# Tesla-Albert/Hybrid-Grid-for-Hexagonal-and-Rectangular-Image-Processing

Measured on AMD Instinct MI355X. Metric: Mpix/s rect→hex→rect+hexconv, 4K batch=128, 1/2/4/8 GPU; %HBM roofline, higher is better.
Workload: dtype bf16

## Files before the change

hybrid-grid-for-hexagonal-and-rectangular-image-processing_amd/csrc/fused4.hip:

```cpp
#include <climits>
#include <cmath>
#include <cstdlib>

#include "fused_kernel.h"

namespace hg {

#ifndef F4_RB_
#define F4_RB_ 30
#endif
#ifndef F4_PD
#define F4_PD 2
#endif
#ifndef F4_WPS
#define F4_WPS 29
#endif
#ifndef F4_ORDER
#define F4_ORDER 0
#endif
#ifndef F4_WPE
#define F4_WPE 3
#endif
#ifndef F4_REV
#define F4_REV 1
#endif
constexpr int F4_GW = 4, F4_THREADS = 256;
constexpr int F4_HL = 8, F4_OWN = 240;
constexpr int F4_RB = F4_RB_;
static_assert(F4_RB % 6 == 0 && F4_RB > 0, "bands are whole 6-step blocks");

typedef unsigned f4_u2 __attribute__((ext_vector_type(2)));

__device__ __forceinline__ void f4_unpack(f4_u2 r, fu_f2& a, fu_f2& b, unsigned hi16) {
    a = fu_f2{__builtin_bit_cast(float, r.x << 16), __builtin_bit_cast(float, r.x & hi16)};
    b = fu_f2{__builtin_bit_cast(float, r.y << 16), __builtin_bit_cast(float, r.y & hi16)};
}

template <int OP>
__global__ __launch_bounds__(F4_THREADS) __attribute__((amdgpu_waves_per_eu(F4_WPE)))
void k_fused4(const __bf16* __restrict__ x, const float* __restrict__ kern,
              const float* __restrict__ bias, __bf16* __restrict__ y, FusedGeom F) {
    constexpr int C = 3, O = 3;
    constexpr int PD = F4_PD;
    static_assert(PD >= 1 && PD <= 4, "raw ring: rows k+2 .. k+1+PD in flight in 6 slots");
    constexpr int RB = F4_RB, NLUT = RB + 2;
    __shared__ float4 lut_all[F4_GW][NLUT];
    const int lane = threadIdx.x & 63;
    const int wslot = __builtin_amdgcn_readfirstlane(threadIdx.x >> 6);
    float4* const lut = lut_all[wslot];
    const int64_t blk = (int64_t)xcd_swizzle(blockIdx.x, gridDim.x);
    const int ngrp = (F.nwin + F4_GW - 1) / F4_GW;
    const int grp = (int)(F4_ORDER == 1 ? (blk / F.nband) % ngrp : blk % ngrp);
    const int band = (int)(F4_ORDER == 1 ? blk % F.nband : (blk / ngrp) % F.nband);
    const int64_t b = blk / ((int64_t)ngrp * F.nband);
    if (b >= F.B) return;
    const int win = grp * F4_GW + wslot;
    const int W0 = win * F4_OWN - F4_HL;
    const int ce = W0 + 4 * lane;
    const int s0 = band * RB;
    const int s1 = min(s0 + RB, F.h2);
    const bool up = F4_REV && (band & 1) && s1 - s0 == RB;

    for (int e = lane; e < NLUT; e += 64) {
        const int r = s0 - 1 + e;
        float4 t = {0.f, 0.f, 0.f, 0.f};
        if (r >= 0 && r < F.h1) {
            const double i_ = axis_at(F.rxs, r) + (double)(F.h - 1) * 0.5;
            const int in = (int)i_;
            const double f = i_ - (double)(float)in;
            const float w0 = (in >= 0 && in < F.h) ? (float)(1.0 - f) : 0.f;
            const float w1 = (in + 1 >= 0 && in + 1 < F.h) ? (float)f : 0.f;
            if (in == r - 1) { t.x = w0; t.y = w1; }
            else if (in == r) { t.y = w0; t.z = w1; }
        }
        lut[e] = t;
    }
    __builtin_amdgcn_s_waitcnt(0xc07f);
    __builtin_amdgcn_wave_barrier();
    int rc;
    {
        bool has_a = false, has_c = false;
        for (int e = lane; e < NLUT; e += 64) {
            const float4 t = lut[e];
            has_a |= t.x != 0.f;
            has_c |= t.z != 0.f;
        }
        const bool any_a = __builtin_amdgcn_ballot_w64(has_a) != 0;
        const bool any_c = __builtin_amdgcn_ballot_w64(has_c) != 0;
        rc = !any_c ? 1 : (!any_a ? 2 : 0);
    }

    float we[2][3], wo[2][3];
#pragma unroll
    for (int k = 0; k < 2; ++k)
#pragma unroll
        for (int s = 0; s < 2; ++s) {
            float* wr = s ? wo[k] : we[k];
            wr[0] = wr[1] = wr[2] = 0.f;
            const int q = ce + 2 * k + s;
            if (q >= 0 && q < F.w1) {
                const double j_ = axis_at(F.rys, q) + (double)(F.w - 1) * 0.5;
                const int jn = (int)j_;
                const double jf = j_ - (double)(float)jn;
#pragma unroll
                for (int kk = -1; kk <= 1; ++kk) {
                    const bool in_w = q + kk >= 0 && q + kk < F.w;
                    if (kk == jn - q && in_w) wr[kk + 1] += (float)(1.0 - jf);
                    if (kk == jn + 1 - q && in_w) wr[kk + 1] += (float)jf;
                }
            }
#pragma unroll
            for (int t = 0; t < 3; ++t) wr[t] *= 0.75f;
        }
    const bool any_l = __builtin_amdgcn_ballot_w64(we[0][0] != 0.f || wo[0][0] != 0.f ||
                                                   we[1][0] != 0.f || wo[1][0] != 0.f) != 0;
    const bool any_r = __builtin_amdgcn_ballot_w64(we[0][2] != 0.f || wo[0][2] != 0.f ||
                                                   we[1][2] != 0.f || wo[1][2] != 0.f) != 0;
    const int cd = !any_r ? 1 : (!any_l ? 2 : 0);

    const bool own = lane >= F4_HL / 4 && lane < (F4_HL + F4_OWN) / 4 && ce >= 0 && ce < F.w2 &&
                     win < F.nwin;

    const int64_t cstride = (int64_t)F.h * F.w, ostride = (int64_t)F.h2 * F.w2;
    const __amdgpu_buffer_rsrc_t xrs = __builtin_amdgcn_make_buffer_rsrc(
        (void*)(x + b * C * cstride), (short)0, (int)(C * cstride * 2), 0x00020000);
    const __amdgpu_buffer_rsrc_t yrs = __builtin_amdgcn_make_buffer_rsrc(
        (void*)(y + b * O * ostride), (short)0, (int)(O * ostride * 2), 0x00020000);
    const int lc = min(max(ce, 0), F.w - 4);
    const unsigned xoff = (unsigned)lc * 2u;
    const unsigned yoff = own ? (unsigned)ce * 2u : 0x80000000u;
    const unsigned xplane = (unsigned)(cstride * 2), yplane = (unsigned)(ostride * 2);
    const unsigned xrow = (unsigned)F.w * 2u, yrow = (unsigned)F.w2 * 2u;
    auto row_off = [&](int r) -> unsigned {
        return (unsigned)__builtin_amdgcn_readfirstlane((int)((unsigned)min(max(r, 0), F.h - 1) * xrow));
    };

    int vz = 0;
    asm volatile("" : "+v"(vz));
    constexpr int NW = O * C * 7, NWP = (NW + 1) / 2;
    constexpr int NWS = F4_WPS < NWP ? F4_WPS : NWP;
    float wk[NW];
#pragma unroll
    for (int i = 0; i < NW; ++i) wk[i] = kern[i + (i / 2 < NWS ? 0 : vz)];
    fu_f2 wkp[NWP];
#pragma unroll
    for (int i = 0; i < NWP; ++i) {
        wkp[i] = fu_f2{wk[2 * i], 2 * i + 1 < NW ? wk[2 * i + 1] : 0.f};
        if (i >= NWS) asm volatile("" : "+v"(wkp[i]));
    }
    float bv[O];
#pragma unroll
    for (int o = 0; o < O; ++o) bv[o] = bias ? bias[o + vz] * 0.75f : 0.f;
    fu_f2 bvp[2];
#pragma unroll
    for (int i = 0; i < 2; ++i) {
        bvp[i] = fu_f2{bv[2 * i], 2 * i + 1 < O ? bv[2 * i + 1] : 0.f};
        asm volatile("" : "+v"(bvp[i]));
    }
    float c13 = 1.f / 3.f;
    asm volatile("" : "+v"(c13));
    const float wn_f = (ce + 4 < F.w2) ? c13 : 0.f;
    const float wp_f = (ce - 1 >= 0) ? c13 : 0.f;
    unsigned hi16 = 0xffff0000u;
    asm volatile("" : "+v"(hi16));

    auto run = [&](auto CDc, auto RCc, auto UPc) {
        constexpr int CD = decltype(CDc)::value;
        constexpr int RC = decltype(RCc)::value;
        constexpr bool UP = decltype(UPc)::value;
        auto row = [&](int k) { return UP ? s1 - 1 - k : s0 + k; };
        auto lut_e = [&](int j) { return UP ? RB - j : j + 1; };
        f4_u2 raw[6][C];
        fu_f2 XA[3][C], XB[3][C];
        fu_f2 ZA[3][O], ZB[3][O];

        auto issue = [&](auto SLc, int r, bool live = true) {
            constexpr int SL = decltype(SLc)::value;
            const unsigned so = row_off(r);
            const unsigned vo = live ? xoff : 0x80000000u;
#pragma unroll
            for (int c = 0; c < C; ++c) raw[SL][c] = __builtin_amdgcn_raw_buffer_load_b64(xrs, vo, so + c * xplane, 0);
        };
        auto convert = [&](auto RSc, auto XSc) {
            constexpr int RS = decltype(RSc)::value, XS = decltype(XSc)::value;
#pragma unroll
            for (int c = 0; c < C; ++c) f4_unpack(raw[RS][c], XA[XS][c], XB[XS][c], hi16);
        };

        auto urow = [&](auto PHc, float4 L, auto CENc, auto BELc) {
            constexpr int PH = decltype(PHc)::value;
            constexpr bool CEN = decltype(CENc)::value, BEL = decltype(BELc)::value;
            constexpr int S0 = fu_mod(PH, 3), S1 = fu_mod(PH + 1, 3), S2 = fu_mod(PH + 2, 3);
            constexpr int XM = UP ? S2 : S0, XQ = UP ? S0 : S2;
            constexpr int PB = UP ? fu_mod(PH + 1, 2) : fu_mod(PH, 2), PC = 1 - PB;
            constexpr int TN = UP ? 5 : 0, TD = UP ? 0 : 5;
            const fu_f2 Lxy = {L.x, L.y}, Lzw = {L.z, L.w};
            fu_sfor<0, C>([&](auto Cc) {
                constexpr int c = decltype(Cc)::value;
                float ue[2], uo[2];
                auto vblend = [&](const fu_f2 (&X)[3][C]) {
                    if constexpr (RC == 1) return fu_pfma<1, false>(Lxy, X[S1][c], fu_pmul<0>(Lxy, X[XM][c]));
                    else if constexpr (RC == 2) return fu_pfma<0, false>(Lzw, X[XQ][c], fu_pmul<1>(Lxy, X[S1][c]));
                    else return fu_pfma<0, false>(Lzw, X[XQ][c], fu_pfma<1, false>(Lxy, X[S1][c], fu_pmul<0>(Lxy, X[XM][c])));
                };
                const fu_f2 VA = vblend(XA), VB = vblend(XB);
                if constexpr (CD == 1) {
                    ue[0] = fmaf(we[0][1], VA.x, we[0][0] * f_prev(VB.y));
                    uo[0] = fmaf(wo[0][1], VA.y, wo[0][0] * VA.x);
                    ue[1] = fmaf(we[1][1], VB.x, we[1][0] * VA.y);
                    uo[1] = fmaf(wo[1][1], VB.y, wo[1][0] * VB.x);
                } else if constexpr (CD == 2) {
                    ue[0] = fmaf(we[0][2], VA.y, we[0][1] * VA.x);
                    uo[0] = fmaf(wo[0][2], VB.x, wo[0][1] * VA.y);
                    ue[1] = fmaf(we[1][2], VB.y, we[1][1] * VB.x);
                    uo[1] = fmaf(wo[1][2], f_next(VA.x), wo[1][1] * VB.y);
                } else {
                    const float pl = f_prev(VB.y), nx = f_next(VA.x);
                    ue[0] = fmaf(we[0][2], VA.y, fmaf(we[0][1], VA.x, we[0][0] * pl));
                    uo[0] = fmaf(wo[0][2], VB.x, fmaf(wo[0][1], VA.y, wo[0][0] * VA.x));
                    ue[1] = fmaf(we[1][2], VB.y, fmaf(we[1][1], VB.x, we[1][0] * VA.y));
                    uo[1] = fmaf(wo[1][2], nx, fmaf(wo[1][1], VB.y, wo[1][0] * VB.x));
                }
                const float nue = f_next(ue[0]);
                const fu_f2 U0[2] = {fu_f2{ue[0], uo[0]}, fu_f2{ue[1], uo[1]}};
                const fu_f2 U1[2] = {fu_f2{uo[0], ue[1]}, fu_f2{uo[1], nue}};
                const fu_f2 Um[2] = {fu_f2{f_prev(uo[1]), ue[0]}, fu_f2{uo[0], ue[1]}};
                const fu_f2 U2[2] = {U0[1], fu_f2{nue, OP == 0 ? f_next(uo[0]) : 0.f}};
                fu_sfor<0, O>([&](auto OOc) {
                    constexpr int o = decltype(OOc)::value;
                    constexpr int j0 = (o * C + c) * 7;
                    auto tapk = [&](auto Tc, fu_f2& zA, fu_f2& zB, int par) {
                        constexpr int j = j0 + decltype(Tc)::value;
                        constexpr bool WS = (j >> 1) < NWS;
                        const int s = fu_tap_shift(decltype(Tc)::value, par, OP);
                        const fu_f2 aA = s == -1 ? Um[0] : (s == 0 ? U0[0] : (s == 1 ? U1[0] : U2[0]));
                        const fu_f2 aB = s == -1 ? Um[1] : (s == 0 ? U0[1] : (s == 1 ? U1[1] : U2[1]));
                        zA = fu_pfma<j & 1, WS>(wkp[j >> 1], aA, zA);
                        zB = fu_pfma<j & 1, WS>(wkp[j >> 1], aB, zB);
                    };
                    if constexpr (c == 0) {
                        constexpr int jb = j0 + TN;
                        constexpr bool WS = (jb >> 1) < NWS;
                        const int s = fu_tap_shift(TN, PB, OP);
                        const fu_f2 aA = s == -1 ? Um[0] : (s == 0 ? U0[0] : (s == 1 ? U1[0] : U2[0]));
                        const fu_f2 aB = s == -1 ? Um[1] : (s == 0 ? U0[1] : (s == 1 ? U1[1] : U2[1]));
                        ZA[S2][o] = fu_pfma_b<jb & 1, o & 1, WS>(wkp[jb >> 1], aA, bvp[o >> 1]);
                        ZB[S2][o] = fu_pfma_b<jb & 1, o & 1, WS>(wkp[jb >> 1], aB, bvp[o >> 1]);
                    } else {
                        tapk(IC<TN>{}, ZA[S2][o], ZB[S2][o], PB);
                    }
                    tapk(IC<TN + 1>{}, ZA[S2][o], ZB[S2][o], PB);
                    if constexpr (CEN) {
                        tapk(IC<2>{}, ZA[S1][o], ZB[S1][o], PC);
                        tapk(IC<3>{}, ZA[S1][o], ZB[S1][o], PC);
                        tapk(IC<4>{}, ZA[S1][o], ZB[S1][o], PC);
                    }
                    if constexpr (BEL) {
                        tapk(IC<TD>{}, ZA[S0][o], ZB[S0][o], PB);
                        tapk(IC<TD + 1>{}, ZA[S0][o], ZB[S0][o], PB);
                    }
                });
            });
        };

        auto out_row = [&](auto PHc, int k) {
            constexpr int PH = decltype(PHc)::value;
            constexpr int S0 = PH % 3;
            constexpr int PAR = UP ? (PH + 1) & 1 : PH & 1;
            const unsigned so = (unsigned)__builtin_amdgcn_readfirstlane((int)((unsigned)row(k) * yrow));
#pragma unroll
            for (int o = 0; o < O; ++o) {
                const fu_f2 zA = ZA[S0][o], zB = ZB[S0][o];
                float o0, o1, o2, o3;
                if constexpr (PAR == 0) {
                    o0 = fmaf(c13, zA.y, zA.x);
                    o1 = fmaf(c13, zB.x, zA.y);
                    o2 = fmaf(c13, zB.y, zB.x);
                    o3 = fmaf(wn_f, f_next(zA.x), zB.y);
                } else {
                    o0 = fmaf(wp_f, f_prev(zB.y), zA.x);
                    o1 = fmaf(c13, zA.x, zA.y);
                    o2 = fmaf(c13, zA.y, zB.x);
                    o3 = fmaf(c13, zB.x, zB.y);
                }
                typedef __bf16 t2v __attribute__((ext_vector_type(2)));
                const f4_u2 v = {__builtin_bit_cast(unsigned, t2v{(__bf16)o0, (__bf16)o1}),
                                 __builtin_bit_cast(unsigned, t2v{(__bf16)o2, (__bf16)o3})};
                __builtin_amdgcn_raw_buffer_store_b64(v, yrs, yoff, so + o * yplane, 0);
            }
        };

        {
            f4_u2 t0[C], t1[C], t2[C];
            const unsigned o0 = row_off(row(-2)), o1 = row_off(row(-1)), o2 = row_off(row(0));
#pragma unroll
            for (int c = 0; c < C; ++c) {
                t0[c] = __builtin_amdgcn_raw_buffer_load_b64(xrs, xoff, o0 + c * xplane, 0);
                t1[c] = __builtin_amdgcn_raw_buffer_load_b64(xrs, xoff, o1 + c * xplane, 0);
                t2[c] = __builtin_amdgcn_raw_buffer_load_b64(xrs, xoff, o2 + c * xplane, 0);
            }
            issue(IC<1>{}, row(1));
#pragma unroll
            for (int i = 0; i < PD; ++i) {
                if (i == 0) issue(IC<2>{}, row(2));
                if (i == 1) issue(IC<3>{}, row(3));
                if (i == 2) issue(IC<4>{}, row(4));
                if (i == 3) issue(IC<5>{}, row(5));
            }
#pragma unroll
            for (int c = 0; c < C; ++c) {
                f4_unpack(t0[c], XA[1][c], XB[1][c], hi16);
                f4_unpack(t1[c], XA[2][c], XB[2][c], hi16);
                f4_unpack(t2[c], XA[0][c], XB[0][c], hi16);
            }
        }
        urow(IC<-2>{}, lut[lut_e(-1)], std::false_type{}, std::false_type{});
        convert(IC<1>{}, IC<1>{});
        urow(IC<-1>{}, lut[lut_e(0)], std::true_type{}, std::false_type{});
        __builtin_amdgcn_s_waitcnt(0x0f70);

        const int n = s1 - s0;
        float4 lnext = lut[lut_e(1)];
        auto step = [&](auto PHc, int k) {
            constexpr int PH = decltype(PHc)::value;
            __builtin_amdgcn_sched_barrier(0);
            convert(IC<(PH + 2) % 6>{}, IC<(PH + 2) % 3>{});
            issue(IC<(PH + 2 + PD) % 6>{}, row(min(k + 2 + PD, n + 1)), k + 2 + PD <= n + 1);
            const float4 L = lnext;
            lnext = lut[min(max(lut_e(k + 2), 0), NLUT - 1)];
            urow(PHc, L, std::true_type{}, std::true_type{});
            out_row(PHc, k);
        };
        auto block6 = [&](int base) {
            step(IC<0>{}, base);
            step(IC<1>{}, base + 1);
            step(IC<2>{}, base + 2);
            step(IC<3>{}, base + 3);
            step(IC<4>{}, base + 4);
            step(IC<5>{}, base + 5);
        };
        int base = 0;
        for (; base + 6 <= n; base += 6) block6(base);
        if constexpr (!UP) {
            if (base < n) {
                step(IC<0>{}, base);
                if (base + 1 < n) {
                    step(IC<1>{}, base + 1);
                    if (base + 2 < n) {
                        step(IC<2>{}, base + 2);
                        if (base + 3 < n) {
                            step(IC<3>{}, base + 3);
                            if (base + 4 < n) step(IC<4>{}, base + 4);
                        }
                    }
                }
            }
        }
    };
    auto dir = [&](auto CDc, auto RCc) {
        if (F4_REV && up) run(CDc, RCc, std::true_type{});
        else run(CDc, RCc, std::false_type{});
    };
    if (cd == 1 && rc == 1) dir(IC<1>{}, IC<1>{});
    else if (cd == 1 && rc == 2) dir(IC<1>{}, IC<2>{});
    else if (cd == 2 && rc == 1) dir(IC<2>{}, IC<1>{});
    else if (cd == 2 && rc == 2) dir(IC<2>{}, IC<2>{});
    else dir(IC<0>{}, IC<0>{});
}

int fused4_try(const void* x, const float* k, const float* bias, void* y, int x_dtype, int y_dtype,
               int C, int O, int G, const FusedGeom& F0, int op, hipStream_t st) {
    if (env_is("HYGRID_FUSED4", "0")) return HG_EUNSUP;
    if (x_dtype != HG_BF16 || y_dtype != HG_BF16 || C != 3 || O != 3 || G != 1) return HG_EUNSUP;
    if ((F0.w % 4) || (F0.w2 % 4) || F0.w < 4) return HG_EUNSUP;
    FusedGeom F = F0;
    F.nwin = (int)((F.w2 + F4_OWN - 1) / F4_OWN);
    F.nband = (int)((F.h2 + F4_RB - 1) / F4_RB);
    const int64_t blocks = F.B * (int64_t)F.nband * ((F.nwin + F4_GW - 1) / F4_GW);
    if (blocks > INT_MAX) return HG_EUNSUP;
    const dim3 grid((unsigned)blocks), blk(F4_THREADS);
    if (op)
        hipLaunchKernelGGL((k_fused4<1>), grid, blk, 0, st, (const __bf16*)x, k, bias, (__bf16*)y, F);
    else
        hipLaunchKernelGGL((k_fused4<0>), grid, blk, 0, st, (const __bf16*)x, k, bias, (__bf16*)y, F);
    return launch_status();
}

}

namespace hg {
void fused4_layout(int* band_rows, int* win_own, int* win_halo) {
    *band_rows = F4_RB;
    *win_own = F4_OWN;
    *win_halo = F4_HL;
}
}
```

Baseline: 406,600.

## Hand-schedule fused row step with packed-FMA asm and DPP lane shifts

Rewrites the per-row inner step of the fused rect→hex→rect kernel as a software-pipelined sequence. Unpacking, vertical blend, horizontal blend, neighbour straddling, conv taps, loads and stores are interleaved across channels and separated by sched_barrier fences. Vertical/horizontal blends and the hex-to-rect output use inline v_pk_fma_f32 asm and DPP wave_shl/shr moves instead of compiler-generated shuffles. The unpack layout changes and the conv taps read only the neighbour values they need. waves_per_eu is pinned to both min and max. The intent is to cut VALU and cross-lane instruction count and hide memory latency, at the cost of fragile hand-written asm and a rigid schedule the compiler cannot adapt.

```diff
diff --git a/hybrid-grid-for-hexagonal-and-rectangular-image-processing_amd/csrc/fused4.hip b/hybrid-grid-for-hexagonal-and-rectangular-image-processing_amd/csrc/fused4.hip
--- a/hybrid-grid-for-hexagonal-and-rectangular-image-processing_amd/csrc/fused4.hip
+++ b/hybrid-grid-for-hexagonal-and-rectangular-image-processing_amd/csrc/fused4.hip
@@ -31,13 +31,126 @@
 
 typedef unsigned f4_u2 __attribute__((ext_vector_type(2)));
 
-__device__ __forceinline__ void f4_unpack(f4_u2 r, fu_f2& a, fu_f2& b, unsigned hi16) {
-    a = fu_f2{__builtin_bit_cast(float, r.x << 16), __builtin_bit_cast(float, r.x & hi16)};
-    b = fu_f2{__builtin_bit_cast(float, r.y << 16), __builtin_bit_cast(float, r.y & hi16)};
-}
+__device__ __forceinline__ void f4_unpack(f4_u2 r, fu_f2& p, fu_f2& q, unsigned hi16) {
+    p = fu_f2{__builtin_bit_cast(float, r.x << 16), __builtin_bit_cast(float, r.y << 16)};
+    q = fu_f2{__builtin_bit_cast(float, r.x & hi16), __builtin_bit_cast(float, r.y & hi16)};
+}
+__device__ __forceinline__ fu_f2 f4_pmul2(fu_f2 w, fu_f2 a) {
+    fu_f2 d;
+    asm("v_pk_mul_f32 %0, %1, %2" : "=v"(d) : "v"(w), "v"(a));
+    return d;
+}
+__device__ __forceinline__ fu_f2 f4_pfma2(fu_f2 w, fu_f2 a, fu_f2 c) {
+    asm("v_pk_fma_f32 %0, %1, %2, %0" : "+v"(c) : "v"(w), "v"(a));
+    return c;
+}
+#define F4_SHR_ " wave_shr:1 row_mask:0xf bank_mask:0xf bound_ctrl:1"
+#define F4_SHL_ " wave_shl:1 row_mask:0xf bank_mask:0xf bound_ctrl:1"
+template <int RC>
+__device__ __forceinline__ fu_f2 f4_vblend(fu_f2 lxy, fu_f2 lzw, fu_f2 xm, fu_f2 x1, fu_f2 xq) {
+    fu_f2 d;
+    if constexpr (RC == 1)
+        asm("v_pk_mul_f32 %0, %1, %2 op_sel_hi:[0,1]\n\t"
+            "v_pk_fma_f32 %0, %1, %3, %0 op_sel:[1,0,0] op_sel_hi:[1,1,1]"
+            : "=&v"(d) : "v"(lxy), "v"(xm), "v"(x1));
+    else if constexpr (RC == 2)
+        asm("v_pk_mul_f32 %0, %1, %3 op_sel:[1,0] op_sel_hi:[1,1]\n\t"
+            "v_pk_fma_f32 %0, %2, %4, %0 op_sel_hi:[0,1,1]"
+            : "=&v"(d) : "v"(lxy), "v"(lzw), "v"(x1), "v"(xq));
+    else
+        asm("v_pk_mul_f32 %0, %1, %3 op_sel_hi:[0,1]\n\t"
+            "v_pk_fma_f32 %0, %1, %4, %0 op_sel:[1,0,0] op_sel_hi:[1,1,1]\n\t"
+            "v_pk_fma_f32 %0, %2, %5, %0 op_sel_hi:[0,1,1]"
+            : "=&v"(d) : "v"(lxy), "v"(lzw), "v"(xm), "v"(x1), "v"(xq));
+    return d;
+}
+__device__ __forceinline__ void f4_hblend_prev(fu_f2 w0q, fu_f2 w1q, float w00, float w01,
+                                               float w10, float w11, fu_f2 vp, fu_f2 vq,
+                                               fu_f2& up, fu_f2& uq) {
+    float ux, uy;
+    asm("v_pk_mul_f32 %0, %3, %5\n\t"
+        "v_mul_f32 %2, %9, %13\n\t"
+        "v_fmac_f32 %2, %10, %12\n\t"
+        "v_mul_f32_dpp %1, %14, %7" F4_SHR_ "\n\t"
+        "v_pk_fma_f32 %0, %4, %6, %0\n\t"
+        "v_fmac_f32 %1, %8, %11"
+        : "=&v"(uq), "=&v"(ux), "=&v"(uy)
+        : "v"(w0q), "v"(w1q), "v"(vp), "v"(vq), "v"(w00), "v"(w01), "v"(w10), "v"(w11),
+          "v"(vp.x), "v"(vp.y), "v"(vq.x), "v"(vq.y));
+    up = fu_f2{ux, uy};
+}
+__device__ __forceinline__ void f4_hblend_next(fu_f2 w1p, fu_f2 w2p, float w01, float w02,
+                                               float w11, float w12, fu_f2 vp, fu_f2 vq,
+                                               fu_f2& up, fu_f2& uq) {
+    float ux, uy;
+    asm("v_pk_mul_f32 %0, %3, %5\n\t"
+        "v_mul_f32 %1, %7, %13\n\t"
+        "v_fmac_f32 %1, %8, %12\n\t"
+        "v_mul_f32 %2, %9, %14\n\t"
+        "v_pk_fma_f32 %0, %4, %6, %0\n\t"
+        "v_fmac_f32_dpp %2, %11, %10" F4_SHL_
+        : "=&v"(up), "=&v"(ux), "=&v"(uy)
+        : "v"(w1p), "v"(w2p), "v"(vp), "v"(vq), "v"(w01), "v"(w02), "v"(w11), "v"(w12),
+          "v"(vp.x), "v"(vp.y), "v"(vq.x), "v"(vq.y));
+    uq = fu_f2{ux, uy};
+}
+template <bool NL, bool NR2>
+__device__ __forceinline__ void f4_straddle(fu_f2 up, fu_f2 uq, fu_f2& ul, fu_f2& ur, fu_f2& ur2) {
+    float rx, ry, lx = 0.f, ly = 0.f, sx = 0.f, sy = 0.f;
+    if constexpr (NR2 && NL)
+        asm("v_mov_b32 %0, %7\n\t"
+            "v_mov_b32 %3, %8\n\t"
+            "v_mov_b32_dpp %1, %6" F4_SHL_ "\n\t"
+            "v_mov_b32_dpp %2, %9" F4_SHR_ "\n\t"
+            "v_mov_b32 %4, %9\n\t"
+            "v_mov_b32_dpp %5, %8" F4_SHL_
+            : "=&v"(rx), "=&v"(ry), "=&v"(lx), "=&v"(ly), "=&v"(sx), "=&v"(sy)
+            : "v"(up.x), "v"(up.y), "v"(uq.x), "v"(uq.y));
+    else if constexpr (NR2)
+        asm("v_mov_b32 %0, %5\n\t"
+            "v_mov_b32 %2, %7\n\t"
+            "v_mov_b32_dpp %1, %4" F4_SHL_ "\n\t"
+            "v_mov_b32_dpp %3, %6" F4_SHL_
+            : "=&v"(rx), "=&v"(ry), "=&v"(sx), "=&v"(sy)
+            : "v"(up.x), "v"(up.y), "v"(uq.x), "v"(uq.y));
+    else
+        asm("v_mov_b32 %0, %5\n\t"
+            "v_mov_b32 %3, %6\n\t"
+            "v_mov_b32_dpp %1, %4" F4_SHL_ "\n\t"
+            "v_mov_b32_dpp %2, %7" F4_SHR_
+            : "=&v"(rx), "=&v"(ry), "=&v"(lx), "=&v"(ly)
+            : "v"(up.x), "v"(up.y), "v"(uq.x), "v"(uq.y));
+    ur = fu_f2{rx, ry};
+    ul = fu_f2{lx, ly};
+    ur2 = fu_f2{sx, sy};
+}
+__device__ __forceinline__ void f4_h2r_even(fu_f2 za, fu_f2 zb, fu_f2 cw, float& o0, float& o1,
+                                            float& o2, float& o3) {
+    fu_f2 d;
+    float a, zby = zb.y;
+    asm("v_pk_fma_f32 %0, %3, %5, %4 op_sel_hi:[0,1,1]\n\t"
+        "v_fma_f32 %1, %9, %7, %8\n\t"
+        "v_fmac_f32_dpp %2, %6, %10" F4_SHL_
+        : "=&v"(d), "=&v"(a), "+v"(zby)
+        : "v"(cw), "v"(za), "v"(zb), "v"(za.x), "v"(za.y), "v"(zb.x), "v"(cw.x), "v"(cw.y));
+    o0 = d.x; o1 = a; o2 = d.y; o3 = zby;
+}
+__device__ __forceinline__ void f4_h2r_odd(fu_f2 za, fu_f2 zb, fu_f2 cw, float& o0, float& o1,
+                                           float& o2, float& o3) {
+    fu_f2 d;
+    float a, zax = za.x;
+    asm("v_pk_fma_f32 %0, %3, %4, %5 op_sel_hi:[0,1,1]\n\t"
+        "v_fma_f32 %1, %9, %7, %8\n\t"
+        "v_fmac_f32_dpp %2, %6, %10" F4_SHR_
+        : "=&v"(d), "=&v"(a), "+v"(zax)
+        : "v"(cw), "v"(za), "v"(zb), "v"(zb.y), "v"(zb.x), "v"(za.y), "v"(cw.x), "v"(cw.y));
+    o0 = zax; o1 = d.x; o2 = a; o3 = d.y;
+}
+#undef F4_SHR_
+#undef F4_SHL_
 
 template <int OP>
-__global__ __launch_bounds__(F4_THREADS) __attribute__((amdgpu_waves_per_eu(F4_WPE)))
+__global__ __launch_bounds__(F4_THREADS) __attribute__((amdgpu_waves_per_eu(F4_WPE, F4_WPE)))
 void k_fused4(const __bf16* __restrict__ x, const float* __restrict__ kern,
               const float* __restrict__ bias, __bf16* __restrict__ y, FusedGeom F) {
     constexpr int C = 3, O = 3;
@@ -117,6 +230,12 @@
     const bool any_r = __builtin_amdgcn_ballot_w64(we[0][2] != 0.f || wo[0][2] != 0.f ||
                                                    we[1][2] != 0.f || wo[1][2] != 0.f) != 0;
     const int cd = !any_r ? 1 : (!any_l ? 2 : 0);
+    fu_f2 WE[3], WO[3];
+#pragma unroll
+    for (int t = 0; t < 3; ++t) {
+        WE[t] = fu_f2{we[0][t], we[1][t]};
+        WO[t] = fu_f2{wo[0][t], wo[1][t]};
+    }
 
     const bool own = lane >= F4_HL / 4 && lane < (F4_HL + F4_OWN) / 4 && ce >= 0 && ce < F.w2 &&
                      win < F.nwin;
@@ -161,6 +280,7 @@
     asm volatile("" : "+v"(c13));
     const float wn_f = (ce + 4 < F.w2) ? c13 : 0.f;
     const float wp_f = (ce - 1 >= 0) ? c13 : 0.f;
+    const fu_f2 c13n = {c13, wn_f}, c13p = {c13, wp_f};
     unsigned hi16 = 0xffff0000u;
     asm volatile("" : "+v"(hi16));
 
@@ -187,108 +307,110 @@
             for (int c = 0; c < C; ++c) f4_unpack(raw[RS][c], XA[XS][c], XB[XS][c], hi16);
         };
 
-        auto urow = [&](auto PHc, float4 L, auto CENc, auto BELc) {
+        auto urow = [&](auto PHc, float4 L, auto CENc, auto BELc, auto&& pre, auto&& mid, auto&& fin,
+                        auto&& put) {
             constexpr int PH = decltype(PHc)::value;
             constexpr bool CEN = decltype(CENc)::value, BEL = decltype(BELc)::value;
             constexpr int S0 = fu_mod(PH, 3), S1 = fu_mod(PH + 1, 3), S2 = fu_mod(PH + 2, 3);
             constexpr int XM = UP ? S2 : S0, XQ = UP ? S0 : S2;
             constexpr int PB = UP ? fu_mod(PH + 1, 2) : fu_mod(PH, 2), PC = 1 - PB;
             constexpr int TN = UP ? 5 : 0, TD = UP ? 0 : 5;
+            constexpr auto reads = [](int s) {
+                bool r = fu_tap_shift(TN, PB, OP) == s || fu_tap_shift(TN + 1, PB, OP) == s;
+                if (BEL) r = r || fu_tap_shift(TD, PB, OP) == s || fu_tap_shift(TD + 1, PB, OP) == s;
+                if (CEN) r = r || fu_tap_shift(2, PC, OP) == s || fu_tap_shift(3, PC, OP) == s ||
+                             fu_tap_shift(4, PC, OP) == s;
+                return r;
+            };
+            constexpr bool NEED_L = reads(-1), NEED_R2 = reads(2);
             const fu_f2 Lxy = {L.x, L.y}, Lzw = {L.z, L.w};
-            fu_sfor<0, C>([&](auto Cc) {
+            fu_f2 VP[C], VQ[C];
+            fu_f2 UP_[C], UQ_[C], UR[C], UL[C], UR2[C];
+            auto fence = [] { __builtin_amdgcn_sched_barrier(0); };
+            auto vblend = [&](auto Cc) {
                 constexpr int c = decltype(Cc)::value;
-                float ue[2], uo[2];
-                auto vblend = [&](const fu_f2 (&X)[3][C]) {
-                    if constexpr (RC == 1) return fu_pfma<1, false>(Lxy, X[S1][c], fu_pmul<0>(Lxy, X[XM][c]));
-                    else if constexpr (RC == 2) return fu_pfma<0, false>(Lzw, X[XQ][c], fu_pmul<1>(Lxy, X[S1][c]));
-                    else return fu_pfma<0, false>(Lzw, X[XQ][c], fu_pfma<1, false>(Lxy, X[S1][c], fu_pmul<0>(Lxy, X[XM][c])));
-                };
-                const fu_f2 VA = vblend(XA), VB = vblend(XB);
+                VP[c] = f4_vblend<RC>(Lxy, Lzw, XA[XM][c], XA[S1][c], XA[XQ][c]);
+                VQ[c] = f4_vblend<RC>(Lxy, Lzw, XB[XM][c], XB[S1][c], XB[XQ][c]);
+            };
+            auto hblend = [&](auto Cc) {
+                constexpr int c = decltype(Cc)::value;
+                const fu_f2 vp = VP[c], vq = VQ[c];
                 if constexpr (CD == 1) {
-                    ue[0] = fmaf(we[0][1], VA.x, we[0][0] * f_prev(VB.y));
-                    uo[0] = fmaf(wo[0][1], VA.y, wo[0][0] * VA.x);
-                    ue[1] = fmaf(we[1][1], VB.x, we[1][0] * VA.y);
-                    uo[1] = fmaf(wo[1][1], VB.y, wo[1][0] * VB.x);
+                    f4_hblend_prev(WO[0], WO[1], we[0][0], we[0][1], we[1][0], we[1][1], vp, vq,
+                                   UP_[c], UQ_[c]);
                 } else if constexpr (CD == 2) {
-                    ue[0] = fmaf(we[0][2], VA.y, we[0][1] * VA.x);
-                    uo[0] = fmaf(wo[0][2], VB.x, wo[0][1] * VA.y);
-                    ue[1] = fmaf(we[1][2], VB.y, we[1][1] * VB.x);
-                    uo[1] = fmaf(wo[1][2], f_next(VA.x), wo[1][1] * VB.y);
+                    f4_hblend_next(WE[1], WE[2], wo[0][1], wo[0][2], wo[1][1], wo[1][2], vp, vq,
+                                   UP_[c], UQ_[c]);
                 } else {
-                    const float pl = f_prev(VB.y), nx = f_next(VA.x);
-                    ue[0] = fmaf(we[0][2], VA.y, fmaf(we[0][1], VA.x, we[0][0] * pl));
-                    uo[0] = fmaf(wo[0][2], VB.x, fmaf(wo[0][1], VA.y, wo[0][0] * VA.x));
-                    ue[1] = fmaf(we[1][2], VB.y, fmaf(we[1][1], VB.x, we[1][0] * VA.y));
-                    uo[1] = fmaf(wo[1][2], nx, fmaf(wo[1][1], VB.y, wo[1][0] * VB.x));
+                    const fu_f2 tl = {we[0][0] * f_prev(vq.y), we[1][0] * vq.x};
+                    UP_[c] = f4_pfma2(WE[2], vq, f4_pfma2(WE[1], vp, tl));
+                    const fu_f2 tq = f4_pfma2(WO[1], vq, f4_pmul2(WO[0], vp));
+                    UQ_[c] = fu_f2{fmaf(wo[0][2], vp.y, tq.x), fmaf(wo[1][2], f_next(vp.x), tq.y)};
                 }
-                const float nue = f_next(ue[0]);
-                const fu_f2 U0[2] = {fu_f2{ue[0], uo[0]}, fu_f2{ue[1], uo[1]}};
-                const fu_f2 U1[2] = {fu_f2{uo[0], ue[1]}, fu_f2{uo[1], nue}};
-                const fu_f2 Um[2] = {fu_f2{f_prev(uo[1]), ue[0]}, fu_f2{uo[0], ue[1]}};
-                const fu_f2 U2[2] = {U0[1], fu_f2{nue, OP == 0 ? f_next(uo[0]) : 0.f}};
+            };
+            auto straddle = [&](auto Cc) {
+                constexpr int c = decltype(Cc)::value;
+                f4_straddle<NEED_L, NEED_R2>(UP_[c], UQ_[c], UL[c], UR[c], UR2[c]);
+            };
+            auto tap = [&](auto SLc, auto PARc, auto Cc, auto Tc, auto BIASc) {
+                constexpr int SL = decltype(SLc)::value, PAR = decltype(PARc)::value;
+                constexpr int c = decltype(Cc)::value, T = decltype(Tc)::value;
+                constexpr int s = fu_tap_shift(T, PAR, OP);
+                const fu_f2 aA = s == -1 ? UL[c] : (s == 0 ? UP_[c] : (s == 1 ? UQ_[c] : UR[c]));
+                const fu_f2 aB = s == -1 ? UP_[c] : (s == 0 ? UQ_[c] : (s == 1 ? UR[c] : UR2[c]));
                 fu_sfor<0, O>([&](auto OOc) {
                     constexpr int o = decltype(OOc)::value;
-                    constexpr int j0 = (o * C + c) * 7;
-                    auto tapk = [&](auto Tc, fu_f2& zA, fu_f2& zB, int par) {
-                        constexpr int j = j0 + decltype(Tc)::value;
-                        constexpr bool WS = (j >> 1) < NWS;
-                        const int s = fu_tap_shift(decltype(Tc)::value, par, OP);
-                        const fu_f2 aA = s == -1 ? Um[0] : (s == 0 ? U0[0] : (s == 1 ? U1[0] : U2[0]));
-                        const fu_f2 aB = s == -1 ? Um[1] : (s == 0 ? U0[1] : (s == 1 ? U1[1] : U2[1]));
-                        zA = fu_pfma<j & 1, WS>(wkp[j >> 1], aA, zA);
-                        zB = fu_pfma<j & 1, WS>(wkp[j >> 1], aB, zB);
-                    };
-                    if constexpr (c == 0) {
-                        constexpr int jb = j0 + TN;
-                        constexpr bool WS = (jb >> 1) < NWS;
-                        const int s = fu_tap_shift(TN, PB, OP);
-                        const fu_f2 aA = s == -1 ? Um[0] : (s == 0 ? U0[0] : (s == 1 ? U1[0] : U2[0]));
-                        const fu_f2 aB = s == -1 ? Um[1] : (s == 0 ? U0[1] : (s == 1 ? U1[1] : U2[1]));
-                        ZA[S2][o] = fu_pfma_b<jb & 1, o & 1, WS>(wkp[jb >> 1], aA, bvp[o >> 1]);
-                        ZB[S2][o] = fu_pfma_b<jb & 1, o & 1, WS>(wkp[jb >> 1], aB, bvp[o >> 1]);
+                    constexpr int j = (o * C + c) * 7 + T;
+                    constexpr bool WS = (j >> 1) < NWS;
+                    if constexpr (decltype(BIASc)::value) {
+                        ZA[SL][o] = fu_pfma_b<j & 1, o & 1, WS>(wkp[j >> 1], aA, bvp[o >> 1]);
+                        ZB[SL][o] = fu_pfma_b<j & 1, o & 1, WS>(wkp[j >> 1], aB, bvp[o >> 1]);
                     } else {
-                        tapk(IC<TN>{}, ZA[S2][o], ZB[S2][o], PB);
-                    }
-                    tapk(IC<TN + 1>{}, ZA[S2][o], ZB[S2][o], PB);
-                    if constexpr (CEN) {
-                        tapk(IC<2>{}, ZA[S1][o], ZB[S1][o], PC);
-                        tapk(IC<3>{}, ZA[S1][o], ZB[S1][o], PC);
-                        tapk(IC<4>{}, ZA[S1][o], ZB[S1][o], PC);
-                    }
-                    if constexpr (BEL) {
-                        tapk(IC<TD>{}, ZA[S0][o], ZB[S0][o], PB);
-                        tapk(IC<TD + 1>{}, ZA[S0][o], ZB[S0][o], PB);
+                        ZA[SL][o] = fu_pfma<j & 1, WS>(wkp[j >> 1], aA, ZA[SL][o]);
+                        ZB[SL][o] = fu_pfma<j & 1, WS>(wkp[j >> 1], aB, ZB[SL][o]);
                     }
                 });
-            });
+            };
+            auto level = [&](auto Lc) {
+                constexpr int l = decltype(Lc)::value;
+                if constexpr (l < 2 * C) {
+                    tap(IC<S2>{}, IC<PB>{}, IC<l / 2>{}, IC<TN + l % 2>{}, std::bool_constant<l == 0>{});
+                    if constexpr (BEL)
+                        tap(IC<S0>{}, IC<PB>{}, IC<l / 2>{}, IC<TD + l % 2>{}, std::false_type{});
+                }
+                if constexpr (CEN)
+                    tap(IC<S1>{}, IC<PC>{}, IC<l / 3>{}, IC<2 + l % 3>{}, std::false_type{});
+            };
+            static_assert(C == 3, "the stage skew below is written out for three channels");
+            fence(); pre(IC<0>{});
+            fence(); vblend(IC<0>{});
+            fence(); pre(IC<1>{});
+            fence(); hblend(IC<0>{}); vblend(IC<1>{});
+            fence(); pre(IC<2>{});
+            fence(); straddle(IC<0>{}); hblend(IC<1>{}); vblend(IC<2>{});
+            fence(); mid(IC<0>{});
+            fence(); level(IC<0>{}); straddle(IC<1>{}); hblend(IC<2>{});
+            fence(); mid(IC<1>{});
+            fence(); level(IC<1>{}); straddle(IC<2>{});
+            fence(); mid(IC<2>{});
+            fence(); level(IC<2>{});
+            fence(); mid(IC<3>{});
+            fence(); level(IC<3>{});
+            fence(); mid(IC<4>{});
+            fence(); level(IC<4>{});
+            fence(); mid(IC<5>{});
+            fence(); level(IC<5>{});
+            fence(); fin();
+            fence(); level(IC<6>{});
+            fence(); put(IC<0>{});
+            fence(); level(IC<7>{});
+            fence(); put(IC<1>{});
+            fence(); level(IC<8>{});
+            fence(); put(IC<2>{});
+            fence();
         };
-
-        auto out_row = [&](auto PHc, int k) {
-            constexpr int PH = decltype(PHc)::value;
-            constexpr int S0 = PH % 3;
-            constexpr int PAR = UP ? (PH + 1) & 1 : PH & 1;
-            const unsigned so = (unsigned)__builtin_amdgcn_readfirstlane((int)((unsigned)row(k) * yrow));
-#pragma unroll
-            for (int o = 0; o < O; ++o) {
-                const fu_f2 zA = ZA[S0][o], zB = ZB[S0][o];
-                float o0, o1, o2, o3;
-                if constexpr (PAR == 0) {
-                    o0 = fmaf(c13, zA.y, zA.x);
-                    o1 = fmaf(c13, zB.x, zA.y);
-                    o2 = fmaf(c13, zB.y, zB.x);
-                    o3 = fmaf(wn_f, f_next(zA.x), zB.y);
-                } else {
-                    o0 = fmaf(wp_f, f_prev(zB.y), zA.x);
-                    o1 = fmaf(c13, zA.x, zA.y);
-                    o2 = fmaf(c13, zA.y, zB.x);
-                    o3 = fmaf(c13, zB.x, zB.y);
-                }
-                typedef __bf16 t2v __attribute__((ext_vector_type(2)));
-                const f4_u2 v = {__builtin_bit_cast(unsigned, t2v{(__bf16)o0, (__bf16)o1}),
-                                 __builtin_bit_cast(unsigned, t2v{(__bf16)o2, (__bf16)o3})};
-                __builtin_amdgcn_raw_buffer_store_b64(v, yrs, yoff, so + o * yplane, 0);
-            }
-        };
+        auto no1 = [](auto) {};
+        auto no0 = [] {};
 
         {
             f4_u2 t0[C], t1[C], t2[C];
@@ -314,22 +436,57 @@
                 f4_unpack(t2[c], XA[0][c], XB[0][c], hi16);
             }
         }
-        urow(IC<-2>{}, lut[lut_e(-1)], std::false_type{}, std::false_type{});
+        urow(IC<-2>{}, lut[lut_e(-1)], std::false_type{}, std::false_type{}, no1, no1, no0, no1);
         convert(IC<1>{}, IC<1>{});
-        urow(IC<-1>{}, lut[lut_e(0)], std::true_type{}, std::false_type{});
+        urow(IC<-1>{}, lut[lut_e(0)], std::true_type{}, std::false_type{}, no1, no1, no0, no1);
         __builtin_amdgcn_s_waitcnt(0x0f70);
 
         const int n = s1 - s0;
         float4 lnext = lut[lut_e(1)];
+        unsigned lso = row_off(row(min(2 + PD, n + 1)));
         auto step = [&](auto PHc, int k) {
             constexpr int PH = decltype(PHc)::value;
-            __builtin_amdgcn_sched_barrier(0);
-            convert(IC<(PH + 2) % 6>{}, IC<(PH + 2) % 3>{});
-            issue(IC<(PH + 2 + PD) % 6>{}, row(min(k + 2 + PD, n + 1)), k + 2 + PD <= n + 1);
+            constexpr int RS = (PH + 2) % 6, XS = (PH + 2) % 3, LS = (PH + 2 + PD) % 6;
+            constexpr int S0 = PH % 3;
+            constexpr int PAR = UP ? (PH + 1) & 1 : PH & 1;
             const float4 L = lnext;
-            lnext = lut[min(max(lut_e(k + 2), 0), NLUT - 1)];
-            urow(PHc, L, std::true_type{}, std::true_type{});
-            out_row(PHc, k);
+            float ov[O][4];
+            unsigned lvo = 0, sso = 0;
+            int nrow = 0;
+            auto pre = [&](auto Cc) {
+                constexpr int c = decltype(Cc)::value;
+                f4_unpack(raw[RS][c], XA[XS][c], XB[XS][c], hi16);
+            };
+            auto mid = [&](auto Ic) {
+                constexpr int i = decltype(Ic)::value;
+                if constexpr (i == 0) {
+                    lvo = k + 2 + PD <= n + 1 ? xoff : 0x80000000u;
+                }
+                if constexpr (i < C)
+                    raw[LS][i] = __builtin_amdgcn_raw_buffer_load_b64(xrs, lvo, lso + i * xplane, 0);
+                if constexpr (i == 3) lnext = lut[min(max(lut_e(k + 2), 0), NLUT - 1)];
+                if constexpr (i == 4) nrow = row(min(k + 3 + PD, n + 1));
+                if constexpr (i == 5) nrow = min(max(nrow, 0), F.h - 1);
+            };
+            auto fin = [&] {
+                lso = (unsigned)__builtin_amdgcn_readfirstlane((int)((unsigned)nrow * xrow));
+                __builtin_amdgcn_sched_barrier(0);
+#pragma unroll
+                for (int o = 0; o < O; ++o) {
+                    if constexpr (PAR == 0) f4_h2r_even(ZA[S0][o], ZB[S0][o], c13n, ov[o][0], ov[o][1], ov[o][2], ov[o][3]);
+                    else f4_h2r_odd(ZA[S0][o], ZB[S0][o], c13p, ov[o][0], ov[o][1], ov[o][2], ov[o][3]);
+                }
+                __builtin_amdgcn_sched_barrier(0);
+                sso = (unsigned)__builtin_amdgcn_readfirstlane((int)((unsigned)row(k) * yrow));
+            };
+            auto put = [&](auto Oc) {
+                constexpr int o = decltype(Oc)::value;
+                typedef __bf16 t2v __attribute__((ext_vector_type(2)));
+                const f4_u2 v = {__builtin_bit_cast(unsigned, t2v{(__bf16)ov[o][0], (__bf16)ov[o][1]}),
+                                 __builtin_bit_cast(unsigned, t2v{(__bf16)ov[o][2], (__bf16)ov[o][3]})};
+                __builtin_amdgcn_raw_buffer_store_b64(v, yrs, yoff, sso + o * yplane, 0);
+            };
+            urow(PHc, L, std::true_type{}, std::true_type{}, pre, mid, fin, put);
         };
         auto block6 = [&](int base) {
             step(IC<0>{}, base);
```

Result: faster. 419,700 (median of 6 runs) (+3.2%).
